# evo-design/evo

Measured on AMD Instinct MI355X. Metric: nucleotides/sec forward scoring, evo-1 7B, higher is better.
Workload: dtype bf16; 1 GPU; evo-1-8k-base scoring, batch 8 x 8,192 nt per GPU (BASELINE configs[1]); batch_per_gpu=8, nt=8192, parallelism=single GPU

## Files before the change

### evo_amd/_build.py

```python
from __future__ import annotations

import os
import shutil
import subprocess
from pathlib import Path

ROOT = Path(__file__).resolve().parent
CSRC = ROOT / "csrc"
LIBDIR = ROOT / "_lib"
LIBNAME = os.environ.get("EVO_AMD_LIBNAME", "libevo_mi355x.so")
ARCH = "gfx950"

EXPORTS = [
    "evo_abi_version", "evo_embed_bf16", "evo_rmsnorm_bf16", "evo_hyena_seg_state", "evo_hyena_carry_scan", "evo_hyena_carry_add",
    "evo_hyena_apply", "evo_hyena_step", "evo_rope_qk_bf16", "evo_attn_fwd_causal_bf16", "evo_attn_decode_bf16",
    "evo_linear_small_m_bf16", "evo_mlp_gate_small_m_bf16", "evo_norm_mlp_gate_small_m_bf16", "evo_norm_linear_small_m_bf16", "evo_hyena_decode_fused_small_m", "evo_linear_mfma_bf16", "evo_mlp_gate_mfma_bf16", "evo_linear_xblk_mfma_bf16", "evo_hyena_ct", "evo_linear_t_mfma_bf16", "evo_rmsnorm_rows_bf16", "evo_gelu_gate_bf16",
    "evo_logprob_entropy", "evo_unembed_logprob_bf16", "evo_unembed_profile_bf16", "evo_rope_append_decode_bf16",
    "evo_linear_mfma_nf_bf16", "evo_linear_xblk_mfma_nf_bf16", "evo_mlp_gate_mfma_nf_bf16", "evo_linear_t_mfma_nf_bf16", "evo_rms_finalize_f32",
    "evo_probe_copy_f4", "evo_probe_mfma_bf16", "evo_pool_rows_bf16", "evo_sample_rows_f32",
    "evo_attn_fwd_prefix_bf16", "evo_attn_prefix_vt_bf16", "evo_attn_decode_prefix_bf16", "evo_rope_append_decode_at_bf16",
]


def lib_path() -> Path:
    return LIBDIR / LIBNAME


def sources():
    return sorted(CSRC.glob("*.hip"))


def _hipcc() -> str:
    for cand in (os.environ.get("HIPCC"), shutil.which("hipcc"), "/opt/rocm/bin/hipcc"):
        if cand and os.path.exists(cand):
            return cand
    raise RuntimeError("hipcc not found: cannot build libevo_mi355x.so")


def is_stale() -> bool:
    out = lib_path()
    if not out.exists():
        return True
    deps = list(sources()) + list(CSRC.glob("*.h")) + [ROOT.parent / "include" / "evo_mi355x.h"]
    newest = max(p.stat().st_mtime for p in deps if p.exists())
    return newest > out.stat().st_mtime


FILE_FLAGS = {"attn_w64.hip": ["-fno-slp-vectorize", "-Wno-unused-value"]}


def _compile_one(args):
    src, obj, verbose = args
    cmd = [_hipcc(), f"--offload-arch={ARCH}", "-O3", "-std=c++17", "-fPIC", "-fno-gpu-rdc", "-Wno-inline-asm"] \
# ... 37 lines not shown
```

### evo_amd/csrc/elementwise.hip

```cpp
#include "common.h"
#include "../../include/evo_mi355x.h"

__global__ __launch_bounds__(256) void embed_kernel(const int64_t* __restrict__ ids, const uint4* __restrict__ w,
                                                    uint4* __restrict__ out, int64_t n_tok, int nvec, int64_t vocab,
                                                    int* __restrict__ bad_flag) {
    int64_t i = (int64_t)blockIdx.x * 256 + threadIdx.x;
    int64_t total = n_tok * nvec;
    for (; i < total; i += (int64_t)gridDim.x * 256) {
        int64_t tok = i / nvec;
        int c = (int)(i - tok * nvec);
        const int64_t id = ids[tok];
        if (id >= 0 && id < vocab) {
            out[i] = w[id * nvec + c];
        } else {
            out[i] = make_uint4(0u, 0u, 0u, 0u);
            if (bad_flag && c == 0) *bad_flag = 1;
        }
    }
}

extern "C" int evo_embed_bf16(const int64_t* ids, const void* weight, void* out, int64_t n_tok, int64_t D,
                              int64_t vocab, int* bad_flag, void* stream) {
    if (D % 8 != 0 || n_tok < 0 || vocab <= 0) return -1;
    if (n_tok == 0) return 0;
    int nvec = (int)(D / 8);
    int64_t total = n_tok * nvec;
    int grid = (int)((total + 255) / 256 < 8192 ? (total + 255) / 256 : 8192);
    hipLaunchKernelGGL(embed_kernel, dim3(grid), dim3(256), 0, (hipStream_t)stream, ids, (const uint4*)weight,
                       (uint4*)out, n_tok, nvec, vocab, bad_flag);
    return evo_launch_status();
}

__device__ __forceinline__ void unpack8(const uint4& v, float* f) {
    f[0] = bf_lo(v.x); f[1] = bf_hi(v.x); f[2] = bf_lo(v.y); f[3] = bf_hi(v.y);
    f[4] = bf_lo(v.z); f[5] = bf_hi(v.z); f[6] = bf_lo(v.w); f[7] = bf_hi(v.w);
}
__device__ __forceinline__ uint4 pack8(const float* f) {
    uint4 v;
    v.x = pack_bf2(f[0], f[1]); v.y = pack_bf2(f[2], f[3]); v.z = pack_bf2(f[4], f[5]); v.w = pack_bf2(f[6], f[7]);
    return v;
}

__device__ __forceinline__ int64_t rms_out_row(int64_t row, int64_t T, int64_t Tp, int64_t Tm, int64_t tail0) {
    if (T == 0) return row;
    const int64_t b = row / T, t = row - b * T;
    return t < Tm ? b * Tp + t : tail0 + b * (T - Tm) + (t - Tm);
}

template <bool HAS_BIAS, int NV>
__global__ __launch_bounds__(256) void rmsnorm_kernel(uint4* __restrict__ x, const uint4* __restrict__ bias,
                                                      const uint4* __restrict__ scale, uint4* __restrict__ out,
                                                      int64_t M, int nvec, float eps, float inv_sqrt_d, int64_t T, int64_t Tp, int64_t Tm, int64_t tail0) {
    const int lane = threadIdx.x & 63;
    const int wave = threadIdx.x >> 6;
    for (int64_t row = (int64_t)blockIdx.x * 4 + wave; row < M; row += (int64_t)gridDim.x * 4) {
        uint4* xr = x + row * nvec;
        uint4 v[NV];
        float ss = 0.f;
#pragma unroll
        for (int i = 0; i < NV; ++i) {
            int idx = lane + 64 * i;
            if (idx < nvec) {
// ... 373 lines not shown
```

### evo_amd/ops.py

```python
from __future__ import annotations

import ctypes
import math
import os
import threading
from typing import Optional, Tuple

import torch

from . import _build

_c = ctypes
_PTR = _c.c_void_p
_I64 = _c.c_int64
_F32 = _c.c_float

_SIGNATURES = {
    "evo_abi_version": ([], _c.c_int),
    "evo_embed_bf16": ([_PTR, _PTR, _PTR, _I64, _I64, _I64, _PTR, _PTR], _c.c_int),
    "evo_rmsnorm_bf16": ([_PTR, _PTR, _PTR, _PTR, _I64, _I64, _F32, _PTR], _c.c_int),
    "evo_hyena_seg_state": ([_PTR, _PTR, _PTR, _PTR, _PTR, _PTR, _PTR, _I64, _I64, _I64, _I64, _I64, _PTR], _c.c_int),
    "evo_hyena_carry_scan": ([_PTR, _PTR, _PTR, _PTR, _I64, _I64, _I64, _I64, _PTR], _c.c_int),
    "evo_hyena_carry_add": ([_PTR, _PTR, _PTR, _I64, _I64, _I64, _I64, _PTR], _c.c_int),
    "evo_hyena_apply": ([_PTR] * 10 + [_I64] * 5 + [_PTR], _c.c_int),
    "evo_hyena_step": ([_PTR] * 9 + [_I64] * 3 + [_PTR], _c.c_int),
    "evo_rope_qk_bf16": ([_PTR, _PTR, _PTR, _I64, _I64, _I64, _I64, _F32, _PTR], _c.c_int),
    "evo_attn_fwd_causal_bf16": ([_PTR] * 4 + [_I64] * 14 + [_F32, _PTR, _PTR], _c.c_int),
    "evo_attn_fwd_prefix_bf16": ([_PTR] * 6 + [_I64] * 16 + [_F32, _PTR, _PTR], _c.c_int),
    "evo_attn_prefix_vt_bf16": ([_PTR] * 2 + [_I64] * 5 + [_PTR], _c.c_int),
    "evo_attn_decode_bf16": ([_PTR] * 4 + [_I64] * 11 + [_PTR] * 3 + [_I64, _F32, _PTR], _c.c_int),
    "evo_linear_small_m_bf16": ([_PTR] * 5 + [_I64] * 3 + [_PTR, _I64, _PTR], _c.c_int),
    "evo_linear_mfma_bf16": ([_PTR] * 5 + [_I64] * 3 + [_PTR], _c.c_int),
    "evo_mlp_gate_mfma_bf16": ([_PTR] * 3 + [_I64] * 3 + [_PTR], _c.c_int),
    "evo_hyena_ct": ([_PTR] * 9 + [_I64] * 13 + [_PTR], _c.c_int),
    "evo_linear_t_mfma_bf16": ([_PTR] * 4 + [_I64] * 3 + [_PTR], _c.c_int),
    "evo_rmsnorm_rows_bf16": ([_PTR, _PTR, _PTR, _PTR, _I64, _I64, _F32, _I64, _I64, _I64, _I64, _PTR], _c.c_int),
    "evo_linear_xblk_mfma_bf16": ([_PTR] * 5 + [_I64] * 3 + [_PTR], _c.c_int),
    "evo_linear_mfma_nf_bf16": ([_PTR] * 7 + [_I64] * 4 + [_PTR], _c.c_int),
    "evo_linear_xblk_mfma_nf_bf16": ([_PTR] * 6 + [_I64] * 4 + [_PTR], _c.c_int),
    "evo_mlp_gate_mfma_nf_bf16": ([_PTR] * 4 + [_I64] * 3 + [_PTR], _c.c_int),
    "evo_linear_t_mfma_nf_bf16": ([_PTR] * 5 + [_I64] * 6 + [_PTR], _c.c_int),
    "evo_rms_finalize_f32": ([_PTR, _I64, _I64, _PTR, _I64, _I64, _I64, _F32, _PTR, _PTR], _c.c_int),
    "evo_probe_copy_f4": ([_PTR, _PTR, _I64, _PTR], _c.c_int),
    "evo_probe_mfma_bf16": ([_PTR, _I64, _I64, _PTR], _c.c_int),
    "evo_mlp_gate_small_m_bf16": ([_PTR] * 3 + [_I64] * 4 + [_PTR], _c.c_int),
    "evo_norm_linear_small_m_bf16": ([_PTR] * 5 + [_I64] * 3 + [_c.c_float, _PTR], _c.c_int),
    "evo_norm_mlp_gate_small_m_bf16": ([_PTR] * 4 + [_I64] * 3 + [_c.c_float, _I64, _PTR], _c.c_int),
    "evo_hyena_decode_fused_small_m": ([_PTR] * 12 + [_I64] * 3 + [_c.c_float, _PTR], _c.c_int),
    "evo_gelu_gate_bf16": ([_PTR, _PTR, _I64, _I64, _PTR], _c.c_int),
    "evo_logprob_entropy": ([_PTR, _I64, _PTR, _PTR, _PTR, _I64, _I64, _PTR], _c.c_int),
    "evo_unembed_logprob_bf16": ([_PTR] * 5 + [_I64] * 3 + [_PTR], _c.c_int),
    "evo_unembed_profile_bf16": ([_PTR] * 3 + [_c.POINTER(_c.c_int32), _I64] + [_PTR] * 3 + [_I64] * 3 + [_PTR], _c.c_int),
    "evo_rope_append_decode_bf16": ([_PTR] * 4 + [_F32] + [_I64] * 7 + [_F32, _PTR], _c.c_int),
    "evo_pool_rows_bf16": ([_PTR, _I64, _I64, _I64, _PTR, _I64, _PTR, _F32, _I64, _I64, _PTR, _PTR, _PTR], _c.c_int),
    "evo_attn_decode_prefix_bf16": ([_PTR] * 4 + [_I64] * 11 + [_PTR] * 3 + [_I64] * 8 + [_PTR] * 4 + [_I64, _I64, _F32, _PTR], _c.c_int),
    "evo_rope_append_decode_at_bf16": ([_PTR] * 4 + [_F32] + [_I64] * 7 + [_F32, _PTR, _PTR], _c.c_int),
    "evo_sample_rows_f32": ([_PTR, _I64, _I64, _PTR, _PTR, _PTR, _PTR, _c.c_uint64] + [_PTR] * 7 + [_I64] * 3 + [_PTR], _c.c_int),
}

_LIB = None
ABI_VERSION = 15
ATTN_GROUP_ROWS = 8


class EvoLibraryError(RuntimeError):
    pass


def load_library(build_if_missing: bool = True) -> ctypes.CDLL:
    global _LIB
    if _LIB is not None:
        return _LIB
    path = _build.lib_path()
    if (not path.exists() or (_build.is_stale() and os.environ.get("EVO_AMD_NO_REBUILD") != "1")) and build_if_missing:
        try:
            _build.build()
        except Exception as e:
            if not path.exists():
                raise EvoLibraryError(f"libevo_mi355x.so is missing and could not be built: {e}") from e
            import warnings
            warnings.warn(f"{path} is older than its sources and the rebuild failed ({e}); loading the stale library "
                          f"(its ABI version is checked below)")
    if not path.exists():
        raise EvoLibraryError(f"{path} not found; run `python -c 'import __graft_entry__ as g; g.build()'`")
    lib = ctypes.CDLL(str(path))
    for name, (argtypes, restype) in _SIGNATURES.items():
        fn = getattr(lib, name, None)
        if fn is None:
            raise EvoLibraryError(f"{path} does not export {name}")
        fn.argtypes = argtypes
        fn.restype = restype
    got = lib.evo_abi_version()
    if got != ABI_VERSION:
        raise EvoLibraryError(f"{path} reports ABI version {got}, this binding needs {ABI_VERSION}: the library was built "
# ... 518 lines not shown
        def sliver(Mm):
            a[Mm:] = self.mlp_gate(x[Mm:], w12, scale, eps, w12g=None if w12 is not None else w12g_folded)
        self._main_then_sliver(M, M - Mm,
                               lambda Mm: self._launch("gemm_gate", "evo_mlp_gate_mfma_nf_bf16", x.data_ptr(), rstd.data_ptr(), w12g_folded.data_ptr(),
                                                       a.data_ptr(), Mm, I, K),
                               sliver)
        return a

    def zt_stream_rows_ok(self, B: int, T: int) -> bool:
        Tm, Tp, Mp, r = self.zt_layout(B, T)
        if r > 0:
            return Tp == Tm and Mp == B * Tm and Tm % 256 == 0
        return Tp == T and Mp == B * T

    def linear_t_rs(self, x: torch.Tensor, rstd: torch.Tensor, w_folded: torch.Tensor, b: Optional[torch.Tensor], w: torch.Tensor,
                    scale: torch.Tensor, eps: float, B: int, T: int, tail: bool = True) -> torch.Tensor:
        Tm, Tp, Mp, r = self.zt_layout(B, T)
        assert self.zt_stream_rows_ok(B, T)
        K = x.shape[1]
        N = w.shape[0]
        if r == 0:
            zt = torch.empty(Mp // 256, N, 256, dtype=torch.bfloat16, device=x.device)
            self._launch("gemm_zt", "evo_linear_t_mfma_nf_bf16", x.data_ptr(), rstd.data_ptr(), w_folded.data_ptr(), _ptr(b), zt.data_ptr(),
                         Mp, N, K, Mp, Mp, 0)
            return zt
        zt = torch.empty(Mp // 256 + (1 if tail else 0), N, 256, dtype=torch.bfloat16, device=x.device)
        self._launch("gemm_zt", "evo_linear_t_mfma_nf_bf16", x.data_ptr(), rstd.data_ptr(), w_folded.data_ptr(), _ptr(b), zt.data_ptr(),
                     Mp, N, K, B * T, Tm, r)
        if tail:
            x_tail = x.view(B, T, K)[:, Tm:].reshape(B * r, K).contiguous()
            self._zt_tail_fill(zt, self.norm_linear(x_tail, scale, eps, w, b), B, r)
        return zt

    def hyena_stage1(self, z, fir_w, fir_b, poles, n_heads, z_halo=None, seg_len=None):
        self._need(z, torch.bfloat16, "hyena z")
        B, T, D3 = z.shape
        D = D3 // 3
        agg, C = self._hyena_seg_state(z, z_halo, fir_w, fir_b, poles, None, n_heads, seg_len)
        s_end = torch.empty(B, D, 8, 2, dtype=torch.float32, device=z.device)
        self._launch("hyena_carry_scan", "evo_hyena_carry_scan", agg.data_ptr(), poles.data_ptr(), None, s_end.data_ptr(), B, T, D, C)
        return (agg, C), torch.view_as_complex(s_end)

    def hyena_stage2(self, z, fir_w, fir_b, poles, residues, dskip, n_heads, stage1, z_halo=None, s0=None):
        agg, C = stage1
        B, T, D3 = z.shape
        D = D3 // 3
        if s0 is not None:
            s0r = torch.view_as_real(s0.to(torch.complex64).contiguous())
            self._launch("hyena_carry_add", "evo_hyena_carry_add", agg.data_ptr(), poles.data_ptr(), s0r.data_ptr(), B, T, D, C)
        return self._hyena_apply(z, z_halo, fir_w, fir_b, poles, residues, dskip, agg, None, n_heads, C)

    def hyena_step(self, z_t: torch.Tensor, fir_state: torch.Tensor, iir_state: torch.Tensor, fir_w, fir_b, poles,
                   residues, dskip, n_heads: int) -> torch.Tensor:
        self._need(z_t, torch.bfloat16, "hyena_step z_t")
        self._need(fir_state, torch.bfloat16, "hyena_step fir_state")
        if iir_state.dtype != torch.complex64 or not iir_state.is_contiguous():
            raise RuntimeError("hyena_step: iir_state must be contiguous complex64")
        B, D3 = z_t.shape
        D = D3 // 3
        y = torch.empty(B, D, dtype=torch.bfloat16, device=z_t.device)
        sr = torch.view_as_real(iir_state)
        _check(self.lib.evo_hyena_step(z_t.data_ptr(), fir_state.data_ptr(), sr.data_ptr(), fir_w.data_ptr(),
                                       fir_b.data_ptr(), poles.data_ptr(), residues.data_ptr(), dskip.data_ptr(),
                                       y.data_ptr(), B, D, n_heads, _stream()), "evo_hyena_step")
        return y

# ... 441 lines not shown
```

### evo_amd/scoring.py

```python
from typing import List, NamedTuple, Sequence, Tuple, Union

import numpy as np
import torch

from .tokenizer import CharLevelTokenizer


def prepare_batch(seqs: List[str], tokenizer: CharLevelTokenizer, prepend_bos: bool = True,
                  device: str = "cuda:0") -> Tuple[torch.Tensor, List[int]]:
    seq_lengths = [len(s) for s in seqs]
    longest = max(seq_lengths)
    bos = int(prepend_bos)
    rows = [np.frombuffer(seq.encode(), dtype=np.uint8) for seq in seqs]
    widths = {bos + r.size + (longest - n) for r, n in zip(rows, seq_lengths)}
    if len(widths) != 1:
        raise RuntimeError("prepare_batch: rows have different token lengths (non-ASCII input?)")
    width = widths.pop()
    ids = np.full((len(seqs), width), tokenizer.pad_id, dtype=np.int64)
    if prepend_bos:
        ids[:, 0] = tokenizer.eod_id
    for i, r in enumerate(rows):
        ids[i, bos:bos + r.size] = r
    return torch.from_numpy(ids).to(device), seq_lengths

# ... 3 lines not shown
    return default_ops()


def logits_to_logprobs(logits: torch.Tensor, input_ids: torch.Tensor, trim_bos: bool = True,
                       bf16_logprobs: bool = False) -> torch.Tensor:
    if trim_bos:
        logits = logits[:, :-1]
        input_ids = input_ids[:, 1:]
    assert logits.shape[1] == input_ids.shape[1]
    B, L, V = logits.shape
    if logits.is_cuda:
        lg = logits.reshape(B * L, V)
        if lg.dtype not in (torch.bfloat16, torch.float32):
            lg = lg.float()
        lp, _ = _ops_for(lg).logprob_entropy(lg.contiguous(), input_ids.reshape(-1).to(lg.device))
        out = lp.view(B, L)
    else:
        out = torch.log_softmax(logits.float(), dim=-1).gather(2, input_ids.unsqueeze(-1).long()).squeeze(-1)
    return out.to(torch.bfloat16) if bf16_logprobs else out


def _fused_tail_ok(model, input_ids) -> bool:
    ops = getattr(model, "ops", None) if hasattr(model, "hidden_states") else None
    if not getattr(model, "has_own_unembed", True) or not isinstance(getattr(getattr(model, "unembed", None), "weight", None), torch.Tensor):
        return False
    return (ops is not None and getattr(ops, "name", "") == "hip-gfx950" and hasattr(ops, "unembed_logprob")
            and ops.unembed_logprob_ok(model.unembed.weight.new_empty(1, model.hidden_size), model.unembed.weight))


def score_logprobs_device(model, input_ids: torch.Tensor, want_entropy: bool = False):
    B, T = input_ids.shape
    if _fused_tail_ok(model, input_ids):
        with torch.no_grad():
            hid = model.hidden_states(input_ids)
            tgt = torch.full((B, T), -1, dtype=torch.int64, device=hid.device)
            tgt[:, :-1] = input_ids[:, 1:].to(hid.device)
            lp, en = model.ops.unembed_logprob(hid, model.unembed.weight, tgt.reshape(-1),
                                               want_logprob=not want_entropy, want_entropy=want_entropy)
        return (None if lp is None else lp.view(B, T)[:, :-1]), (None if en is None else en.view(B, T)[:, :-1])
    logits, _ = model(input_ids)
    if not want_entropy:
        return logits_to_logprobs(logits, input_ids, trim_bos=True), None
    logits = logits[:, :-1]
    L, V = logits.shape[1], logits.shape[2]
    if logits.is_cuda:
        lg = logits.reshape(B * L, V).contiguous()
        _, ent = _ops_for(lg).logprob_entropy(lg, None, want_logprob=False, want_entropy=True)
        return None, ent.view(B, L)
    lsm = torch.log_softmax(logits.float(), dim=-1)
    return None, -(lsm.exp() * lsm).sum(-1)


def _reduce(logprobs: np.ndarray, seq_lengths: List[int], reduce_method: str) -> List[float]:
    if reduce_method == "mean":
        fn = np.mean
    elif reduce_method == "sum":
        fn = np.sum
    else:
        raise ValueError(f"Invalid reduce_method {reduce_method}")
    return [fn(logprobs[i][: seq_lengths[i]]) for i in range(len(seq_lengths))]


def score_sequences(seqs: List[str], model, tokenizer: CharLevelTokenizer, reduce_method: str = "mean",
                    device: str = "cuda:0") -> List[float]:
    if reduce_method not in ("mean", "sum"):
        raise ValueError(f"Invalid reduce_method {reduce_method}")
    input_ids, seq_lengths = prepare_batch(seqs, tokenizer, device=device, prepend_bos=True)
# ... 26 lines not shown


def profile_token_ids(tokens: Union[str, Sequence[int]] = "ACGT", vocab: int = 512) -> Tuple[int, ...]:
    if isinstance(tokens, (str, bytes)):
        raw = tokens.encode("utf-8") if isinstance(tokens, str) else tokens
        if isinstance(tokens, str) and len(raw) != len(tokens):
            raise ValueError(f"tokens: {tokens!r} holds a non-ASCII character (one character must be one byte id)")
        ids = list(raw)
    else:
        if isinstance(tokens, torch.Tensor):
            tokens = tokens.tolist()
        try:
            tokens = list(tokens)
            ids = [int(t) for t in tokens]
        except (TypeError, ValueError) as e:
            raise ValueError(f"tokens: expected an ASCII string or a sequence of ints, got {tokens!r}") from e
        if any(i != t for i, t in zip(ids, tokens)):
            raise ValueError(f"tokens: expected integer ids, got {tokens!r}")
    if not 1 <= len(ids) <= PROFILE_MAX_TOKENS:
        raise ValueError(f"tokens: expected 1 to {PROFILE_MAX_TOKENS} tokens, got {len(ids)}")
    for i in ids:
        if not 0 <= i < vocab:
            raise ValueError(f"tokens: id {i} is outside [0, {vocab})")
    if len(set(ids)) != len(ids):
        raise ValueError(f"tokens: a token is given twice in {tokens!r}")
    return tuple(ids)


def score_profile_device(model, input_ids: torch.Tensor, token_ids):
    ids = profile_token_ids(token_ids)
    B, T = input_ids.shape
    if _fused_tail_ok(model, input_ids) and hasattr(model.ops, "unembed_profile"):
        with torch.no_grad():
            hid = model.hidden_states(input_ids)
            tgt = torch.full((B, T), -1, dtype=torch.int64, device=hid.device)
            tgt[:, :-1] = input_ids[:, 1:].to(hid.device)
            sl, lp, en = model.ops.unembed_profile(hid, model.unembed.weight, ids, tgt.reshape(-1))
        return lp.view(B, T)[:, :-1], en.view(B, T)[:, :-1], sl.view(B, T, len(ids))[:, :-1]
    with torch.no_grad():
        logits, _ = model(input_ids)
        lsm = torch.log_softmax(logits[:, :-1].float(), dim=-1)
        lp = lsm.gather(2, input_ids[:, 1:].to(lsm.device).unsqueeze(-1).long()).squeeze(-1)
        en = -(lsm.exp() * lsm).sum(-1)
        sl = lsm.index_select(2, torch.tensor(ids, dtype=torch.int64, device=lsm.device))
    return lp, en, sl


def position_profiles(seqs: List[str], model, tokenizer: CharLevelTokenizer, tokens: Union[str, Sequence[int]] = "ACGT",
                      device: str = "cuda:0") -> List[PositionProfile]:
    ids = profile_token_ids(tokens)
    if len(seqs) == 0:
        raise ValueError("position_profiles: no sequences")
    input_ids, seq_lengths = prepare_batch(seqs, tokenizer, device=device, prepend_bos=True)
    with torch.inference_mode():
        lp, en, sl = score_profile_device(model, input_ids, ids)
    lp, en, sl = lp.float().cpu().numpy(), en.float().cpu().numpy(), sl.float().cpu().numpy()
    out = [PositionProfile(lp[i][:n].copy(), en[i][:n].copy(), sl[i][:n].copy(), ids) for i, n in enumerate(seq_lengths)]
    assert all(len(s) == len(p.logprob) for s, p in zip(seqs, out))
    return out


def substitution_scores(profile: PositionProfile) -> np.ndarray:
    return profile.token_logprobs - profile.logprob[:, None]


def predicted_tokens(profile: PositionProfile) -> np.ndarray:
    return np.asarray(profile.tokens, dtype=np.int64)[profile.token_logprobs.argmax(-1)]
# ... 203 lines not shown
```

### evo_amd/sh/model.py

```python
from __future__ import annotations

import math
import weakref
from typing import Dict, List, Optional, Tuple

import torch
import torch.nn as nn

from ..ops import HipOps
from .cache import InferenceParams, RecurrentInferenceParams
from .utils import dotdict


def _cfg(config, key, default):
    v = config.get(key, None) if isinstance(config, dict) else getattr(config, key, None)
    return default if v is None else v


class _Params(nn.Module):

    def __init__(self, **shapes):
        super().__init__()
        for name, (shape, dtype) in shapes.items():
            self.register_parameter(name, nn.Parameter(torch.empty(*shape, dtype=dtype), requires_grad=False))
# ... 96 lines not shown
        self.norm = _Params(scale=((D,), bf)) if bool(_cfg(c, "final_norm", True)) else None
        self.unembed = _Unembed(self, self.embedding_layer.weight)
        blocks = []
        for i in range(self.num_layers):
            if i in self.attn_layer_idxs:
                blocks.append(_AttentionBlock(D, self.inner_size, self.head_dim))
            else:
                blocks.append(_HyenaBlock(D, self.inner_size, self.state_size, self.short_filter_length))
        self.blocks = nn.ModuleList(blocks)
        self._ops = ops
        self._packed = False
        self._rot_cache: Dict[Tuple[int, int, str], Tuple[torch.Tensor, torch.Tensor]] = {}

    def load_state_dict(self, state_dict, strict: bool = True, assign: bool = True):
        own = dict(self.named_parameters(remove_duplicate=False))
        own.update(dict(self.named_buffers(remove_duplicate=False)))
        missing = [k for k in own if k not in state_dict]
        unexpected = [k for k in state_dict if k not in own]
        if "unembed.weight" in missing and "embedding_layer.weight" in state_dict:
            missing.remove("unembed.weight")
        if strict and (missing or unexpected):
            raise RuntimeError(f"Error(s) in loading state_dict for StripedHyena: missing keys {missing}, "
                               f"unexpected keys {unexpected}")
        if getattr(self, "_norms_folded", False):
            raise RuntimeError("load_state_dict on a model that holds one folded weight set (fold_norms_): build a fresh StripedHyena")
        for k, t in state_dict.items():
            if k not in own or k == "unembed.weight":
                continue
            if tuple(own[k].shape) != tuple(t.shape):
                raise RuntimeError(f"size mismatch for {k}: checkpoint {tuple(t.shape)} vs model {tuple(own[k].shape)}")
            own[k].data = t.detach()
        self._packed = False
        self._rot_cache.clear()
        from torch.nn.modules.module import _IncompatibleKeys
        return _IncompatibleKeys(missing, unexpected)

    def to_bfloat16_except_poles_residues(self):
        for k, p in self.named_parameters():
            if k.endswith("poles") or k.endswith("residues"):
                p.data = p.data.to(torch.float32)
            else:
                p.data = p.data.to(torch.bfloat16)
        for _, b in self.named_buffers():
            b.data = b.data.to(torch.float32)
        self._packed = False

    def _apply(self, fn, recurse=True):
        out = super()._apply(fn, recurse)
        self._packed = False
        self._rot_cache.clear()
        return out

    @property
    def device(self):
        return self.embedding_layer.weight.device

    @property
    def ops(self):
        if self._ops is None:
            from ..ops import default_ops
            self._ops = default_ops()
        return self._ops

    def _pack(self):
        if getattr(self, "_norms_folded", False):
            raise RuntimeError("this StripedHyena holds ONE folded weight set (fold_norms_): its derived tensors cannot be rebuilt from the "
                               "parameters -- moving / re-typing / re-loading needs a fresh model")
        self._pack_impl()

    def _pack_impl(self):
        for blk in self.blocks:
            l1, l2, l3 = blk.mlp.l1.weight, blk.mlp.l2.weight, blk.mlp.l3.weight
            inner, D_ = l1.shape
            ipad = ((inner + 255) // 256) * 256 if inner >= 1024 else inner
            w12 = l1.data.new_zeros(2 * ipad, D_)
            w12[:inner] = l1.data
            w12[ipad:ipad + inner] = l2.data
            w3 = l3.data.new_zeros(D_, ipad)
            w3[:, :inner] = l3.data
            l1.data = w12[:inner]
            l2.data = w12[ipad:ipad + inner]
            l3.data = w3[:, :inner]
            blk.mlp._w12 = w12
            blk.mlp._w3 = w3
            blk.mlp._w12g = None
            blk.mlp._w12g_f = None
            if isinstance(blk, _HyenaBlock):
                blk._wp_f = None
            else:
                blk.inner_mha_cls._wqkv_f = None
            blk.mlp._w12g_ok = (2 * ipad) % 256 == 0 and ipad % 32 == 0 and D_ % 64 == 0 and D_ >= 128
            if isinstance(blk, _HyenaBlock):
                f = blk.filter
                D = self.hidden_size
                f._fir_w = f.short_filter_weight.data.reshape(3 * D, self.short_filter_length).contiguous()
                f._poles = f.poles.data.reshape(D, self.state_size, 2).float().contiguous()
                f._residues = f.residues.data.reshape(D, self.state_size, 2).float().contiguous()
                f._mfma_tab = None
                f._tab_prec = None
        self._packed = True

    def prepare(self, prefill: bool = True) -> "StripedHyena":
        with torch.inference_mode(False), torch.no_grad():
            if not self._packed and not getattr(self, "_norms_folded", False):
                self._pack()
            if prefill:
                nf = getattr(self.ops, "fuse_norm", False) and hasattr(self.ops, "fold_norm_scale") and self.blocks[0].mlp._w12g_ok
                for blk in self.blocks:
                    if getattr(self, "_norms_folded", False):
                        pass
                    elif nf:
                        self._folded(blk.mlp, "_w12g_f", blk.mlp._w12, blk.post_norm.scale, gate=True)
                        if isinstance(blk, _HyenaBlock):
                            self._folded(blk, "_wp_f", blk.projections.weight, blk.pre_norm.scale)
                        else:
                            self._folded(blk.inner_mha_cls, "_wqkv_f", blk.inner_mha_cls.Wqkv.weight, blk.pre_norm.scale)
                    else:
                        self._gate_pack(blk, 1 << 20)
                    if isinstance(blk, _HyenaBlock) and hasattr(self.ops, "hyena_ct") and self._table_ok(blk):
                        self._mfma_table(blk)
        return self

    def fold_norms_(self) -> "StripedHyena":
        if getattr(self, "_norms_folded", False):
            return self
        ops = self.ops
        with torch.inference_mode(False), torch.no_grad():
            if not self._packed:
                self._pack()
            for blk in self.blocks:
                mlp = blk.mlp
                inner = mlp.l1.weight.shape[0]
                w12f = HipOps.fold_norm_scale(mlp._w12, blk.post_norm.scale.data)
                if mlp._w12g_ok and hasattr(ops, "pack_gate_weights"):
                    mlp._w12g = ops.pack_gate_weights(w12f)
                    mlp._w12 = None
                    mlp._l12_shape = (inner, w12f.shape[1])
                    mlp.l1.weight.data = w12f.new_empty(0)
                    mlp.l2.weight.data = w12f.new_empty(0)
                else:
                    ipad = w12f.shape[0] // 2
                    mlp._w12 = w12f
                    mlp._w12g = None
                    mlp.l1.weight.data = w12f[:inner]
                    mlp.l2.weight.data = w12f[ipad:ipad + inner]
                mlp._w12g_f = None
                del w12f
                if isinstance(blk, _HyenaBlock):
                    blk.projections.weight.data = HipOps.fold_norm_scale(blk.projections.weight.data, blk.pre_norm.scale.data)
                    blk._wp_f = None
                else:
                    mha = blk.inner_mha_cls
                    mha.Wqkv.weight.data = HipOps.fold_norm_scale(mha.Wqkv.weight.data, blk.pre_norm.scale.data)
                    mha._wqkv_f = None
                blk.pre_norm.scale.data = torch.ones_like(blk.pre_norm.scale.data)
                blk.post_norm.scale.data = torch.ones_like(blk.post_norm.scale.data)
            self._norms_folded = True
            self._dgraph = None
        return self

    def release_unused_weight_copies(self) -> int:
        before = self.resident_bytes()
        fold = getattr(self.ops, "fuse_norm", False)
        for blk in self.blocks:
            if getattr(self, "_norms_folded", False):
                break
            if fold and getattr(blk.mlp, "_w12g_f", None) is not None:
                blk.mlp._w12g = None
            if not fold:
                blk.mlp._w12g_f = None
                if isinstance(blk, _HyenaBlock):
                    blk._wp_f = None
                else:
                    blk.inner_mha_cls._wqkv_f = None
        return before - self.resident_bytes()

    def state_dict(self, *args, **kwargs):
        sd = super().state_dict(*args, **kwargs)
        if getattr(self, "_norms_folded", False):
            prefix = kwargs.get("prefix", args[1] if len(args) > 1 else "")
            for i, blk in enumerate(self.blocks):
                mlp = blk.mlp
                if mlp._w12 is None:
                    inner, K = mlp._l12_shape
                    g = mlp._w12g.view(-1, 2, 32, K)
                    sd[f"{prefix}blocks.{i}.mlp.l1.weight"] = g[:, 0].reshape(-1, K)[:inner]
                    sd[f"{prefix}blocks.{i}.mlp.l2.weight"] = g[:, 1].reshape(-1, K)[:inner]
        return sd

    def resident_bytes(self) -> int:
        seen, total = set(), 0

        def add(t):
            nonlocal total
            if isinstance(t, torch.Tensor) and t.numel():
                st = t.untyped_storage()
                key = (st.data_ptr(), st.nbytes())
                if key not in seen:
                    seen.add(key)
                    total += st.nbytes()
        for mod in self.modules():
            for t in list(mod._parameters.values()) + list(mod._buffers.values()):
                add(t)
            for k, v in vars(mod).items():
                if k.startswith("_") and isinstance(v, torch.Tensor):
                    add(v)
        return total

# ... 118 lines not shown
            a = ops.mlp_gate(n2, blk.mlp._w12, w12g=blk.mlp._w12g)
        ops.linear_residual_(x2d, a, blk.mlp._w3)

    def _mfma_hyena_ok(self, B: int, T: int) -> bool:
        ops = self.ops
        D, H = self.hidden_size, self.num_heads
        if not getattr(ops, "hyena_mfma", False) or not hasattr(ops, "hyena_ct") or D != H * 128:
            return False
        return T >= 32 and B * T >= 256

    def _mfma_table(self, blk):
        f = blk.filter
        if getattr(f, "_mfma_tab", None) is None or f._mfma_tab.device != blk.projections.weight.device:
            from ..hyena_tables import mfma_operand_table
            f._mfma_tab = mfma_operand_table(f._poles, f._residues, f.D.data)
        return f._mfma_tab

    def _table_ok(self, blk) -> bool:
        f = blk.filter
        if not getattr(self.ops, "hyena_table_guard", True):
            return True
        if getattr(f, "_tab_prec", None) is None:
            from ..hyena_tables import table_precision
            f._tab_prec = float(table_precision(f._poles, f._residues, f.D.data).max())
        from ..hyena_tables import TABLE_TOL
        return f._tab_prec <= TABLE_TOL

    def _hyena_ct_ok(self, x2d, blk, B, T) -> bool:
        ops = self.ops
        w = blk.projections.weight
        return (getattr(ops, "hyena_ct_flag", False) and hasattr(ops, "hyena_ct") and x2d.is_cuda and w.dtype == torch.bfloat16
                and w.is_contiguous() and ops.zt_shape_ok(B, T, w.shape[0], w.shape[1]))

    def _hyena_block(self, i, blk, x2d, B, T, cache: Optional[RecurrentInferenceParams], mask=None, rs=None):
        ops = self.ops
        D, H = self.hidden_size, self.num_heads
        f = blk.filter
        have_state = cache is not None and i in cache.fir_state_dict
        K1 = self.short_filter_length - 1
        if have_state and T == 1:
            y = ops.hyena_decode_fused(x2d, blk.pre_norm.scale, self.eps, blk.projections.weight, blk.projections.bias,
                                       cache.fir_state_dict[i], cache.state_dict[i], f._fir_w, f.short_filter_bias,
                                       f._poles, f._residues, f.D, H)
        elif mask is None and self._mfma_hyena_ok(B, T) and self._hyena_ct_ok(x2d, blk, B, T) and self._table_ok(blk):
            table = self._mfma_table(blk)
            nf = self._nf_ok(B * T, mask)
            pb = None if blk.projections.bias is None else blk.projections.bias.data
            Tm, _, _, r_tail = ops.zt_layout(B, T)
            split = (cache is None and r_tail == 1 and getattr(ops, "hyena_tail_split", False) and HipOps.fused_rows_ok(B, D)
                     and pb is not None)
            if nf and rs is not None and ops.zt_stream_rows_ok(B, T):
                wp_f = self._folded(blk, "_wp_f", blk.projections.weight, blk.pre_norm.scale)
                zt = ops.linear_t_rs(x2d, rs, wp_f, pb, blk.projections.weight.data, blk.pre_norm.scale, self.eps, B, T, tail=not split)
            else:
                xp = ops.rmsnorm_rows(x2d, blk.pre_norm.scale, self.eps, B, T)
                zt = ops.linear_t(xp, blk.projections.weight.data, pb, B, T, tail=not split)
            yb = ops.yblk_empty(B * T, D, zt.device)
            if split:
                y, state = ops.hyena_ct(zt, B, T, f._fir_w, f.short_filter_bias, table, H, want_state=True, poles=f._poles, y_blk=yb,
                                        main_only=True)
                ix = self._tail_split_index(B, T, zt.device)
                fir = zt[ix["zblk"], :, 256 - K1:].contiguous()
                x_tail = x2d.view(B, T, D)[:, Tm].contiguous()
                y_tail = ops.hyena_decode_fused(x_tail, blk.pre_norm.scale, self.eps, blk.projections.weight, blk.projections.bias, fir, state,
                                                f._fir_w, f.short_filter_bias, f._poles, f._residues, f.D, H)
                yb[ix["yblk"], :, ix["yrow"], :] = y_tail.view(B, D // 16, 16)
            elif cache is None:
                y = ops.hyena_ct(zt, B, T, f._fir_w, f.short_filter_bias, table, H, y_blk=yb)
            else:
                halo = s0 = None
                if have_state:
                    halo = cache.fir_state_dict[i].transpose(1, 2).contiguous()
                    s0 = cache.state_dict[i]
                y, state = ops.hyena_ct(zt, B, T, f._fir_w, f.short_filter_bias, table, H, z_halo=halo, s0=s0,
                                        want_state=True, poles=f._poles, y_blk=yb)
                cache.fir_state_dict[i] = ops.zt_rows(zt, B, T, T - K1, K1).transpose(1, 2).contiguous()
                cache.state_dict[i] = state
            if nf:
                return self._mlp_residual_rs_(blk, x2d, self._mixer_out_rs_(blk, x2d, y, blk.out_filter_dense.weight, blk.out_filter_dense.bias))
            self._mlp_residual_(blk, x2d, self._mixer_out_(blk, x2d, y, blk.out_filter_dense.weight, blk.out_filter_dense.bias), None)
            return None
        else:
            z = ops.norm_linear(x2d, blk.pre_norm.scale, self.eps, blk.projections.weight, blk.projections.bias)
            if mask is not None:
# ... 104 lines not shown
                else:
                    a = ops.attention(q, k, v, off, **ak).view(B * T, D)
        if nf:
            return self._mlp_residual_rs_(blk, x2d, self._mixer_out_rs_(blk, x2d, a, mha.out_proj.weight, mha.out_proj.bias))
        self._mlp_residual_(blk, x2d, self._mixer_out_(blk, x2d, a, mha.out_proj.weight, mha.out_proj.bias, mfma=True),
                            None if mask is None else mask[0])
        return None

    max_rows_per_pass = 160 * 1024

    def _row_groups(self, B: int, T: int):
        cap = max(1, self.max_rows_per_pass // T)

        def fits(p):
            r = (p * T) % 256
            return r == 0 or HipOps.fused_rows_ok(r, 4096)

        if B <= cap and (fits(B) or B * T < 65536):
            return [B]
        n0 = (B + cap - 1) // cap

        def split(n):
            q, r = divmod(B, n)
            return [q + 1] * r + [q] * (n - r)

        n = n0
        while n <= B and (B // n) * T >= 32768:
            g = split(n)
            if all(fits(p) for p in set(g)):
                return g
            n += 1
        return split(n0)

    def hidden_states(self, x: torch.Tensor, inference_params_dict=None, padding_mask=None) -> torch.Tensor:
        if not self._packed:
            self._pack()
        if x.dim() != 2:
            raise ValueError("input_ids must be [batch, length]")
        B, T = x.shape
        ops = self.ops
        if padding_mask is not None and tuple(padding_mask.shape) != (B, T):
            raise ValueError(f"padding_mask must be [batch, length] = {(B, T)}, got {tuple(padding_mask.shape)}")
        groups = self._row_groups(B, T) if inference_params_dict is None else [B]
        if len(groups) > 1:
            out, b0 = None, 0
            for nb in groups:
                pm = None if padding_mask is None else padding_mask[b0:b0 + nb]
                hg = self.hidden_states(x[b0:b0 + nb], None, pm)
                if out is None:
                    out = torch.empty(B * T, hg.shape[1], dtype=hg.dtype, device=hg.device)
                out[b0 * T:(b0 + nb) * T] = hg
                b0 += nb
            return out
        h = ops.embed(x.to(self.device), self.embedding_layer.weight)
        mask = None
        if padding_mask is not None:
            pm = padding_mask.to(self.device) != 0
            mask = (pm.reshape(B * T, 1).to(h.dtype), pm.to(torch.uint8).contiguous())
        mha_c = inference_params_dict["mha"] if inference_params_dict is not None else None
        hy_c = inference_params_dict["hyena"] if inference_params_dict is not None else None
        dyn = T == 1 and mha_c is not None and getattr(mha_c, "pos_tensor", None) is not None
        if dyn and not hasattr(ops, "rope_append_decode"):
            mha_c._rot_dyn = self._rotary_dyn(mha_c.pos_tensor)
        try:
            self._run_blocks(h, B, T, mha_c, hy_c, mask)
        finally:
            if dyn:
                mha_c._rot_dyn = None
        if self.norm is not None:
            h = ops.rmsnorm(h, None, self.norm.scale, self.eps)
        return h

    def _run_blocks(self, h: torch.Tensor, B: int, T: int, mha_c, hy_c, mask, stop: Optional[int] = None, after_block=None) -> None:
        stop = self.num_layers if stop is None else stop
        rs = None
        taps = getattr(self, "block_taps", None)
        tap_idxs = getattr(self, "block_tap_idxs", None)
        for i in range(stop):
            blk = self.blocks[i]
            if taps is not None and (tap_idxs is None or i in tap_idxs):
                taps.append(h.clone())
            if isinstance(blk, _AttentionBlock):
                rs = self._attn_block(i, blk, h, B, T, mha_c, mask, rs)
            else:
                rs = self._hyena_block(i, blk, h, B, T, hy_c, mask, rs)
            if after_block is not None:
                after_block(i, h)
        if stop == self.num_layers and taps is not None and (tap_idxs is None or self.num_layers in tap_idxs):
            taps.append(h.clone())

    @torch.no_grad()
    def embeddings(self, input_ids: torch.Tensor, layers, pooling: str = "mean", start: int = 1, lengths=None,
                   padding_mask=None, inference_params_dict=None) -> Dict:
        from ..embeddings import check_pooling, normalize_layers
        if padding_mask is not None:
            raise ValueError("embeddings: padding_mask is not supported (pass the true lengths instead: pads are never pooled)")
        if inference_params_dict is not None:
            raise ValueError("embeddings: an inference cache is not supported (embeddings are a stateless forward)")
        if not self.embedding_layer.weight.is_cuda:
            raise RuntimeError(f"embeddings: the model's weights are on {self.embedding_layer.weight.device}; move the model to the GPU")
        layers = normalize_layers(layers, self.num_layers)
        check_pooling(pooling)
        if input_ids.dim() != 2:
            raise ValueError("input_ids must be [batch, length]")
        B, T = input_ids.shape
        if lengths is None:
            lengths = [T - start] * B
        lengths = [int(n) for n in lengths]
        if len(lengths) != B:
            raise ValueError(f"embeddings: {len(lengths)} lengths for a batch of {B}")
        if start < 0 or any(n < 1 or start + n > T for n in lengths):
            raise ValueError(f"embeddings: every row needs 1 <= length and start + length <= T = {T} (start {start}, lengths {lengths})")
        if not self._packed:
            self._pack()
        ops = self.ops
        D = self.hidden_size
        dev = self.device
        blocks = [l for l in layers if l != "final"]
# ... 140 lines not shown
```

### include/evo_mi355x.h

```cpp
#ifndef EVO_MI355X_H
#define EVO_MI355X_H

#include <stdint.h>

#ifdef __cplusplus
extern "C" {
#endif

#define EVO_ABI_VERSION 15
int evo_abi_version(void);

int evo_embed_bf16(const int64_t* ids, const void* weight, void* out,
                   int64_t n_tok, int64_t D, int64_t vocab, int* bad_flag, void* stream);

int evo_rmsnorm_bf16(void* x, const void* bias, const void* scale, void* out,
                     int64_t M, int64_t D, float eps, void* stream);

int evo_hyena_seg_state(const void* z, const void* z_halo, const void* fir_w, const void* fir_b,
                        const float* poles, float* agg, const uint8_t* mask,
                        int64_t B, int64_t T, int64_t D, int64_t n_heads, int64_t seg_len, void* stream);
int evo_hyena_carry_scan(float* agg, const float* poles, const float* s0, float* s_final,
                         int64_t B, int64_t T, int64_t D, int64_t seg_len, void* stream);
int evo_hyena_carry_add(float* agg, const float* poles, const float* s0,
                        int64_t B, int64_t T, int64_t D, int64_t seg_len, void* stream);
int evo_hyena_apply(const void* z, const void* z_halo, const void* fir_w, const void* fir_b,
                    const float* poles, const float* residues, const void* dskip,
                    const float* agg, void* y, const uint8_t* mask,
                    int64_t B, int64_t T, int64_t D, int64_t n_heads, int64_t seg_len, void* stream);

int evo_hyena_ct(const void* zt, const void* z_halo, const void* fir_w, const void* fir_b, const void* table, void* y,
                 const float* s0, float* s_out, const float* poles, int64_t B, int64_t T, int64_t D, int64_t n_heads,
                 int64_t zt_pitch, int64_t row_pitch, int64_t zt_row0, int64_t tail_T, int64_t tail_pos0, int64_t state_only,
                 int64_t y_blocked_rows, int64_t y_row0, int64_t y_row_pitch, void* stream);

int evo_linear_xblk_mfma_bf16(const void* x_blk, const void* w, const void* bias, const void* residual, void* y,
                              int64_t M, int64_t N, int64_t K, void* stream);

int evo_linear_t_mfma_bf16(const void* x, const void* w, const void* bias, void* zt, int64_t Mp, int64_t N, int64_t K, void* stream);

int evo_rmsnorm_rows_bf16(void* x, const void* bias, const void* scale, void* out, int64_t M, int64_t D, float eps,
                          int64_t T, int64_t Tp, int64_t Tm, int64_t tail0, void* stream);

int evo_hyena_step(const void* z_t, void* fir_state, float* iir_state,
                   const void* fir_w, const void* fir_b, const float* poles, const float* residues,
                   const void* dskip, void* y, int64_t B, int64_t D, int64_t n_heads, void* stream);

int evo_rope_qk_bf16(void* qkv, const float* cos_t, const float* sin_t,
                     int64_t B, int64_t T, int64_t H, int64_t hd, float q_scale, void* stream);

int evo_rope_append_decode_bf16(void* qkv, void* kv, const int64_t* pos, const float* inv_freq, float scaling,
                                int64_t B, int64_t H, int64_t hd, int64_t kv_sb, int64_t kv_st, int64_t kv_sw, int64_t kv_sh,
                                float q_scale, void* stream);
int evo_rope_append_decode_at_bf16(void* qkv, void* kv, const int64_t* pos, const float* inv_freq, float scaling,
                                   int64_t B, int64_t H, int64_t hd, int64_t kv_sb, int64_t kv_st, int64_t kv_sw, int64_t kv_sh,
                                   float q_scale, const int64_t* widx, void* stream);

int evo_attn_fwd_causal_bf16(const void* q, const void* k, const void* v, void* o,
                             int64_t B, int64_t H, int64_t Tq, int64_t Tk, int64_t q_pos0,
                             int64_t q_sb, int64_t q_st, int64_t q_sh,
                             int64_t k_sb, int64_t k_st, int64_t k_sh,
                             int64_t v_sb, int64_t v_st, int64_t v_sh,
                             float softmax_scale, void* vt_ws, void* stream);

int evo_attn_fwd_prefix_bf16(const void* q, const void* k, const void* v, const void* k_pre, const void* vt_pre, void* o,
                             int64_t B, int64_t H, int64_t Tq, int64_t P,
                             int64_t q_sb, int64_t q_st, int64_t q_sh,
                             int64_t k_sb, int64_t k_st, int64_t k_sh,
                             int64_t v_sb, int64_t v_st, int64_t v_sh,
                             int64_t kp_st, int64_t kp_sh, int64_t vtp_row,
                             float softmax_scale, void* vt_ws, void* stream);
int evo_attn_prefix_vt_bf16(const void* v_pre, void* vt_pre, int64_t P, int64_t H, int64_t vp_st, int64_t vp_sh, int64_t vt_row,
                            void* stream);

int evo_attn_decode_bf16(const void* q, const void* k, const void* v, void* o,
// ... 80 lines not shown
```

Baseline: 109,100 nt/s.

## Replace first Hyena block input projection with precomputed per-token lookup table

Layer 0's input is just the embedding of each token, so embedding, RMSNorm and the input projection depend only on the token id. The change builds a per-block table of projected outputs for every vocabulary entry, caches it with the weights, and gathers from it with a new kernel that writes the blocked zt layout directly. This skips the full-sequence GEMM and norm for the first Hyena block during scoring. The cost is extra table memory (N x vocab), invalidation logic when weights change, and a strided gather kernel.

```diff
diff --git a/evo_amd/_build.py b/evo_amd/_build.py
--- a/evo_amd/_build.py
+++ b/evo_amd/_build.py
@@ -19,6 +19,7 @@
     "evo_linear_mfma_nf_bf16", "evo_linear_xblk_mfma_nf_bf16", "evo_mlp_gate_mfma_nf_bf16", "evo_linear_t_mfma_nf_bf16", "evo_rms_finalize_f32",
     "evo_probe_copy_f4", "evo_probe_mfma_bf16", "evo_pool_rows_bf16", "evo_sample_rows_f32",
     "evo_attn_fwd_prefix_bf16", "evo_attn_prefix_vt_bf16", "evo_attn_decode_prefix_bf16", "evo_rope_append_decode_at_bf16",
+    "evo_embed_proj_zt_bf16",
 ]
 
 
diff --git a/evo_amd/csrc/elementwise.hip b/evo_amd/csrc/elementwise.hip
--- a/evo_amd/csrc/elementwise.hip
+++ b/evo_amd/csrc/elementwise.hip
@@ -28,6 +28,54 @@
     int grid = (int)((total + 255) / 256 < 8192 ? (total + 255) / 256 : 8192);
     hipLaunchKernelGGL(embed_kernel, dim3(grid), dim3(256), 0, (hipStream_t)stream, ids, (const uint4*)weight,
                        (uint4*)out, n_tok, nvec, vocab, bad_flag);
+    return evo_launch_status();
+}
+
+__global__ __launch_bounds__(256) void embed_proj_zt_kernel(const int64_t* __restrict__ ids, const uint16_t* __restrict__ table,
+                                                            const uint16_t* __restrict__ bias, uint4* __restrict__ zt, int64_t Tm,
+                                                            int64_t row_skip, int N, int vocab, int* __restrict__ bad_flag) {
+    const int lane = threadIdx.x & 63;
+    const int wave = __builtin_amdgcn_readfirstlane(threadIdx.x >> 6);
+    const int half = lane >> 5;
+    const int col = lane & 31;
+    const int64_t blk = blockIdx.y;
+    const int64_t b = blk * 256 / Tm;
+    const int64_t* src = ids + blk * 256 + b * row_skip + col * 8;
+    uint32_t off[8];
+    unsigned bad = 0;
+#pragma unroll
+    for (int e = 0; e < 8; ++e) {
+        const int64_t v = src[e];
+        const bool ok = v >= 0 && v < vocab;
+        off[e] = (uint32_t)(half * vocab) + (ok ? (uint32_t)v : 0u);
+        bad |= ok ? 0u : 1u << e;
+    }
+    if (bad && bad_flag && blockIdx.x == 0 && wave == 0) *bad_flag = 1;
+    const int c0 = (int)blockIdx.x * 256 + wave * 64;
+    uint4* dst = zt + (blk * N + c0 + half) * 32 + col;
+#pragma unroll 4
+    for (int i = 0; i < 32; ++i) {
+        const uint16_t* row = table + (int64_t)(c0 + 2 * i) * vocab;
+        uint32_t h[8];
+#pragma unroll
+        for (int e = 0; e < 8; ++e) h[e] = row[off[e]];
+        if (bad) {
+            const uint32_t fill = bias ? f_to_bf(0.f + bf_to_f(bias[c0 + 2 * i + half])) : 0u;
+#pragma unroll
+            for (int e = 0; e < 8; ++e) h[e] = (bad >> e & 1u) ? fill : h[e];
+        }
+        dst[(int64_t)i * 64] = make_uint4(h[0] | h[1] << 16, h[2] | h[3] << 16, h[4] | h[5] << 16, h[6] | h[7] << 16);
+    }
+}
+
+extern "C" int evo_embed_proj_zt_bf16(const int64_t* ids, const void* table, const void* bias, void* zt, int64_t B, int64_t Tm,
+                                      int64_t row_skip, int64_t N, int64_t vocab, int* bad_flag, void* stream) {
+    if (B < 0 || Tm <= 0 || Tm % 256 != 0 || row_skip < 0 || N <= 0 || N % 256 != 0 || vocab <= 0 || N * vocab > 0x7fffffff) return -1;
+    const int64_t blocks = B * Tm / 256;
+    if (N / 256 > 65535 || blocks * N * 512 >= 0xfffffff0LL) return -1;
+    if (blocks == 0) return 0;
+    hipLaunchKernelGGL(embed_proj_zt_kernel, dim3((unsigned)(N / 256), (unsigned)blocks), dim3(256), 0, (hipStream_t)stream, ids,
+                       (const uint16_t*)table, (const uint16_t*)bias, (uint4*)zt, Tm, row_skip, (int)N, (int)vocab, bad_flag);
     return evo_launch_status();
 }
 
diff --git a/evo_amd/ops.py b/evo_amd/ops.py
--- a/evo_amd/ops.py
+++ b/evo_amd/ops.py
@@ -56,10 +56,11 @@
     "evo_attn_decode_prefix_bf16": ([_PTR] * 4 + [_I64] * 11 + [_PTR] * 3 + [_I64] * 8 + [_PTR] * 4 + [_I64, _I64, _F32, _PTR], _c.c_int),
     "evo_rope_append_decode_at_bf16": ([_PTR] * 4 + [_F32] + [_I64] * 7 + [_F32, _PTR, _PTR], _c.c_int),
     "evo_sample_rows_f32": ([_PTR, _I64, _I64, _PTR, _PTR, _PTR, _PTR, _c.c_uint64] + [_PTR] * 7 + [_I64] * 3 + [_PTR], _c.c_int),
+    "evo_embed_proj_zt_bf16": ([_PTR] * 4 + [_I64] * 5 + [_PTR, _PTR], _c.c_int),
 }
 
 _LIB = None
-ABI_VERSION = 15
+ABI_VERSION = 16
 ATTN_GROUP_ROWS = 8
 
 
@@ -644,6 +645,39 @@
             self._zt_tail_fill(zt, self.norm_linear(x_tail, scale, eps, w, b), B, r)
         return zt
 
+    def embed_proj_ok(self, B: int, T: int, V: int, N: int, K: int) -> bool:
+        Tm, Tp, Mp, r = self.zt_layout(B, T)
+        return (V % 256 == 0 and N * V < 2 ** 31 and self.zt_shape_ok(1, V, N, K) and self.zt_shape_ok(B, T, N, K)
+                and Tp == Tm and Mp == B * Tm and Tm % 256 == 0)
+
+    def embed_proj_table(self, emb: torch.Tensor, scale: torch.Tensor, eps: float, w: torch.Tensor, b: Optional[torch.Tensor]) -> torch.Tensor:
+        V, D = emb.shape
+        assert V % 256 == 0 and self.zt_layout(1, V) == (V, V, V, 0)
+        saved = getattr(self._xpad, "entry", None)
+        try:
+            self._xpad.entry = None
+            zt = self.linear_t(self.rmsnorm_rows(emb.contiguous(), scale, eps, 1, V), w, b, 1, V)
+        finally:
+            self._xpad.entry = saved
+        return zt.permute(1, 0, 2).reshape(w.shape[0], V).contiguous()
+
+    def embed_proj_zt(self, ids: torch.Tensor, table: torch.Tensor, b: Optional[torch.Tensor], B: int, T: int) -> torch.Tensor:
+        Tm, Tp, Mp, r = self.zt_layout(B, T)
+        N, V = table.shape
+        assert Tp == Tm and Mp == B * Tm and Tm % 256 == 0
+        if tuple(ids.shape) != (B, T):
+            raise RuntimeError(f"embed_proj_zt: ids must be [{B}, {T}], got {tuple(ids.shape)}")
+        if not ids.is_cuda or ids.dtype != torch.int64 or ids.stride(1) != 1 or (B > 1 and ids.stride(0) < T):
+            raise RuntimeError("embed_proj_zt: ids must be a device int64 matrix with contiguous rows")
+        self._check_address(ids.data_ptr(), "embed_proj_zt ids", 8)
+        pitch = ids.stride(0) if B > 1 else T
+        self._need(table, torch.bfloat16, "embed_proj_zt table")
+        if b is not None:
+            self._need(b, torch.bfloat16, "embed_proj_zt bias")
+        zt = torch.empty(Mp // 256, N, 256, dtype=torch.bfloat16, device=table.device)
+        self._launch("embed_proj_zt", "evo_embed_proj_zt_bf16", ids.data_ptr(), table.data_ptr(), _ptr(b), zt.data_ptr(), B, Tm, pitch - Tm, N, V, None)
+        return zt
+
     def hyena_stage1(self, z, fir_w, fir_b, poles, n_heads, z_halo=None, seg_len=None):
         self._need(z, torch.bfloat16, "hyena z")
         B, T, D3 = z.shape
diff --git a/evo_amd/scoring.py b/evo_amd/scoring.py
--- a/evo_amd/scoring.py
+++ b/evo_amd/scoring.py
@@ -59,7 +59,7 @@
     B, T = input_ids.shape
     if _fused_tail_ok(model, input_ids):
         with torch.no_grad():
-            hid = model.hidden_states(input_ids)
+            hid = model.hidden_states(input_ids, embed_proj_table=True)
             tgt = torch.full((B, T), -1, dtype=torch.int64, device=hid.device)
             tgt[:, :-1] = input_ids[:, 1:].to(hid.device)
             lp, en = model.ops.unembed_logprob(hid, model.unembed.weight, tgt.reshape(-1),
@@ -152,7 +152,7 @@
     B, T = input_ids.shape
     if _fused_tail_ok(model, input_ids) and hasattr(model.ops, "unembed_profile"):
         with torch.no_grad():
-            hid = model.hidden_states(input_ids)
+            hid = model.hidden_states(input_ids, embed_proj_table=True)
             tgt = torch.full((B, T), -1, dtype=torch.int64, device=hid.device)
             tgt[:, :-1] = input_ids[:, 1:].to(hid.device)
             sl, lp, en = model.ops.unembed_profile(hid, model.unembed.weight, ids, tgt.reshape(-1))
diff --git a/evo_amd/sh/model.py b/evo_amd/sh/model.py
--- a/evo_amd/sh/model.py
+++ b/evo_amd/sh/model.py
@@ -152,6 +152,7 @@
             own[k].data = t.detach()
         self._packed = False
         self._rot_cache.clear()
+        self._drop_embed_proj_table()
         from torch.nn.modules.module import _IncompatibleKeys
         return _IncompatibleKeys(missing, unexpected)
 
@@ -169,6 +170,7 @@
         out = super()._apply(fn, recurse)
         self._packed = False
         self._rot_cache.clear()
+        self._drop_embed_proj_table()
         return out
 
     @property
@@ -216,6 +218,7 @@
                 f._fir_w = f.short_filter_weight.data.reshape(3 * D, self.short_filter_length).contiguous()
                 f._poles = f.poles.data.reshape(D, self.state_size, 2).float().contiguous()
                 f._residues = f.residues.data.reshape(D, self.state_size, 2).float().contiguous()
+                blk._ep_table = None
                 f._mfma_tab = None
                 f._tab_prec = None
         self._packed = True
@@ -275,6 +278,7 @@
                     mha._wqkv_f = None
                 blk.pre_norm.scale.data = torch.ones_like(blk.pre_norm.scale.data)
                 blk.post_norm.scale.data = torch.ones_like(blk.post_norm.scale.data)
+            self._drop_embed_proj_table()
             self._norms_folded = True
             self._dgraph = None
         return self
@@ -282,6 +286,7 @@
     def release_unused_weight_copies(self) -> int:
         before = self.resident_bytes()
         fold = getattr(self.ops, "fuse_norm", False)
+        self._drop_embed_proj_table()
         for blk in self.blocks:
             if getattr(self, "_norms_folded", False):
                 break
@@ -294,6 +299,11 @@
                 else:
                     blk.inner_mha_cls._wqkv_f = None
         return before - self.resident_bytes()
+
+    def _drop_embed_proj_table(self) -> None:
+        for blk in getattr(self, "blocks", ()):
+            if getattr(blk, "_ep_table", None) is not None:
+                blk._ep_table = None
 
     def state_dict(self, *args, **kwargs):
         sd = super().state_dict(*args, **kwargs)
@@ -478,7 +488,23 @@
         return (getattr(ops, "hyena_ct_flag", False) and hasattr(ops, "hyena_ct") and x2d.is_cuda and w.dtype == torch.bfloat16
                 and w.is_contiguous() and ops.zt_shape_ok(B, T, w.shape[0], w.shape[1]))
 
-    def _hyena_block(self, i, blk, x2d, B, T, cache: Optional[RecurrentInferenceParams], mask=None, rs=None):
+    def _embed_proj_ok(self, blk, B: int, T: int) -> bool:
+        ops = self.ops
+        w = blk.projections.weight
+        return (hasattr(ops, "embed_proj_zt") and self.embedding_layer.weight.dtype == torch.bfloat16
+                and ops.embed_proj_ok(B, T, self.vocab_size, w.shape[0], w.shape[1]))
+
+    def _embed_proj_table(self, blk) -> torch.Tensor:
+        w = blk.projections.weight
+        tab = getattr(blk, "_ep_table", None)
+        if tab is None or tab.device != w.device:
+            with torch.inference_mode(False), torch.no_grad():
+                tab = self.ops.embed_proj_table(self.embedding_layer.weight.data, blk.pre_norm.scale.data, self.eps, w.data,
+                                                None if blk.projections.bias is None else blk.projections.bias.data)
+            blk._ep_table = tab
+        return tab
+
+    def _hyena_block(self, i, blk, x2d, B, T, cache: Optional[RecurrentInferenceParams], mask=None, rs=None, ids=None):
         ops = self.ops
         D, H = self.hidden_size, self.num_heads
         f = blk.filter
@@ -495,7 +521,9 @@
             Tm, _, _, r_tail = ops.zt_layout(B, T)
             split = (cache is None and r_tail == 1 and getattr(ops, "hyena_tail_split", False) and HipOps.fused_rows_ok(B, D)
                      and pb is not None)
-            if nf and rs is not None and ops.zt_stream_rows_ok(B, T):
+            if ids is not None and i == 0 and cache is None and (r_tail == 0 or split) and self._embed_proj_ok(blk, B, T):
+                zt = ops.embed_proj_zt(ids, self._embed_proj_table(blk), pb, B, T)
+            elif nf and rs is not None and ops.zt_stream_rows_ok(B, T):
                 wp_f = self._folded(blk, "_wp_f", blk.projections.weight, blk.pre_norm.scale)
                 zt = ops.linear_t_rs(x2d, rs, wp_f, pb, blk.projections.weight.data, blk.pre_norm.scale, self.eps, B, T, tail=not split)
             else:
@@ -666,7 +694,7 @@
             n += 1
         return split(n0)
 
-    def hidden_states(self, x: torch.Tensor, inference_params_dict=None, padding_mask=None) -> torch.Tensor:
+    def hidden_states(self, x: torch.Tensor, inference_params_dict=None, padding_mask=None, embed_proj_table: bool = False) -> torch.Tensor:
         if not self._packed:
             self._pack()
         if x.dim() != 2:
@@ -686,7 +714,8 @@
                 out[b0 * T:(b0 + nb) * T] = hg
                 b0 += nb
             return out
-        h = ops.embed(x.to(self.device), self.embedding_layer.weight)
+        x = x.to(self.device)
+        h = ops.embed(x, self.embedding_layer.weight)
         mask = None
         if padding_mask is not None:
             pm = padding_mask.to(self.device) != 0
@@ -697,7 +726,8 @@
         if dyn and not hasattr(ops, "rope_append_decode"):
             mha_c._rot_dyn = self._rotary_dyn(mha_c.pos_tensor)
         try:
-            self._run_blocks(h, B, T, mha_c, hy_c, mask)
+            ids0 = x.to(torch.int64) if embed_proj_table and inference_params_dict is None and mask is None else None
+            self._run_blocks(h, B, T, mha_c, hy_c, mask, ids0=ids0)
         finally:
             if dyn:
                 mha_c._rot_dyn = None
@@ -705,7 +735,7 @@
             h = ops.rmsnorm(h, None, self.norm.scale, self.eps)
         return h
 
-    def _run_blocks(self, h: torch.Tensor, B: int, T: int, mha_c, hy_c, mask, stop: Optional[int] = None, after_block=None) -> None:
+    def _run_blocks(self, h: torch.Tensor, B: int, T: int, mha_c, hy_c, mask, stop: Optional[int] = None, after_block=None, ids0=None) -> None:
         stop = self.num_layers if stop is None else stop
         rs = None
         taps = getattr(self, "block_taps", None)
@@ -717,7 +747,7 @@
             if isinstance(blk, _AttentionBlock):
                 rs = self._attn_block(i, blk, h, B, T, mha_c, mask, rs)
             else:
-                rs = self._hyena_block(i, blk, h, B, T, hy_c, mask, rs)
+                rs = self._hyena_block(i, blk, h, B, T, hy_c, mask, rs, ids=ids0 if i == 0 else None)
             if after_block is not None:
                 after_block(i, h)
         if stop == self.num_layers and taps is not None and (tap_idxs is None or self.num_layers in tap_idxs):
diff --git a/include/evo_mi355x.h b/include/evo_mi355x.h
--- a/include/evo_mi355x.h
+++ b/include/evo_mi355x.h
@@ -7,7 +7,7 @@
 extern "C" {
 #endif
 
-#define EVO_ABI_VERSION 15
+#define EVO_ABI_VERSION 16
 int evo_abi_version(void);
 
 int evo_embed_bf16(const int64_t* ids, const void* weight, void* out,
@@ -40,6 +40,9 @@
 
 int evo_rmsnorm_rows_bf16(void* x, const void* bias, const void* scale, void* out, int64_t M, int64_t D, float eps,
                           int64_t T, int64_t Tp, int64_t Tm, int64_t tail0, void* stream);
+
+int evo_embed_proj_zt_bf16(const int64_t* ids, const void* table, const void* bias, void* zt, int64_t B, int64_t Tm,
+                           int64_t row_skip, int64_t N, int64_t vocab, int* bad_flag, void* stream);
 
 int evo_hyena_step(const void* z_t, void* fir_state, float* iir_state,
                    const void* fir_w, const void* fir_b, const float* poles, const float* residues,
```

Result: no change. 109,800 nt/s, median of 6 (+0.6%).
